# neptune-ai/open-solution-salt-identification

Hardware: AMD Instinct MI355X
Metric: training images/sec, U-Net ResNet34 101x101 (pad->128) bs32/GPU (higher is better)
Workload: dtype bf16; 1 GPU; architectures.unet.UNetResNet(34, hypercolumn) 128x128 (101 resized+edge-padded) batch 32/GPU, lovasz loss, Adam lr1e-4 L2 1e-4, train-mode BN; global_batch=32, parallelism=dp1

## Files before the change

### include/saltnet.h

```cpp
#ifndef SALTNET_H
#define SALTNET_H
#include <stdint.h>

#ifdef __cplusplus
extern "C" {
#endif

#define SALT_F32 0
#define SALT_BF16 1

#define SALT_OK 0
#define SALT_E_BADARG -1
#define SALT_E_UNSUPPORTED -2
#define SALT_E_LDS -3

#define SALT_MAX_TAPS 16

typedef struct {
    void* p;
    int B;
    int H;
    int W;
    int C;
    int cs;
// ... 14 lines not shown
    int in_step;
    int pad_mode;
    salt_view y;
    int OH;
    int OW;
    int out_step;
    int out_oy;
    int out_ox;
    const float* bias;
    const float* scale;
    const float* shift;
    int relu;
    int accumulate;
    float* stats;
    float* stats_cnt;
    int stats_part0;
    int cfg;
    void* strip;
    int strip_cs;
    int fold_top;
    int fold_bottom;
    int fold_left;
    int fold_right;
    salt_view bnb_y;
    salt_view bnb_a;
    const float* bnb_mean;
    const float* bnb_invstd;
    const float* bnb_gamma;
    const float* bnb_beta;
    float* bnb_partials;
    int bnb_relu;
    int nphase;
    int64_t w_phase_elems;
    const void* fin;
    double* fin_acc;
    uint32_t* fin_ticket;
    const void* bnb_fin;
    double* bnb_acc;
    uint32_t* bnb_ticket;
    salt_view res;
    const float* in_scale;
    const float* in_shift;
    int in_relu;
    const void* in_fin;
    const double* in_fin_acc;
    int64_t y_plane;
    int64_t x_plane;
} salt_conv_args;
int salt_conv(const salt_conv_args*, void* stream);
int salt_conv_stats_parts(const salt_conv_args*);
int salt_conv_kernel_id(const salt_conv_args*);
int salt_conv_tile_shape(const salt_conv_args*);

typedef struct {
    int dtype;
    salt_view p;
    salt_view q;
    int ntaps;
    int tap_dy[SALT_MAX_TAPS];
    int tap_dx[SALT_MAX_TAPS];
    int q_step;
    int pad_mode;
    float* partials;
    int nsplit;
    int64_t q_plane;
} salt_conv_wgrad_args;
// ... 715 lines not shown
```

### open-solution-salt-identification_amd/csrc/conv_mfma.hip

```cpp
#include <cstdlib>
#include <type_traits>
#include "common.h"
#ifndef SALT_K1_DBG
#define SALT_K1_DBG 0
#endif
#ifndef SALT_K1_FAST_STORE
#define SALT_K1_FAST_STORE 1
#endif

namespace {

struct ConvKP {
    const void* x; const void* w; void* y;
    const float* bias; const float* scale; const float* shift;
    float* stats; float* stats_cnt;
    int B, H, W, Cin, x_cs;
    int Cout, y_cs, OHf, OWf, OH, OW, out_step, out_oy, out_ox;
    int ntaps; int tap_off[SALT_MAX_TAPS];
    int in_step, pad_mode, min_dy, min_dx;
    int th_log2, tw_log2, nb;
    int gen, tw, th, twth;
    unsigned tw_magic, twth_magic;
    int hh, hw;
    int tiles_y, tiles_x;
    int nchunk, a_bytes;
    int relu, accumulate, stats_part0;
    void* strip; int strip_cs, fold_top, fold_bottom, fold_left, fold_right;
    int nphase, m_tiles_ph; int64_t w_phase_elems;
    int fold_fused, ox_shift;
    unsigned hhw_magic, hw_magic;
    int m_tiles, n_tiles;
    int vt;
    int nbuf;
    int no_perm8;
    int y_small;
    const void* bnb_y; const void* bnb_a; int bnb_cs, bnb_acs, bnb_relu;
    const float* bnb_mean; const float* bnb_invstd; const float* bnb_gamma; const float* bnb_beta; float* bnb_partials;
    const void* res; int res_cs;
    BnFin fin; BnbFin bnbf;
    const float* in_scale; const float* in_shift; int in_relu, in_tab_off; BnFin in_fin;
};

template <typename T> struct Mma;
template <> struct Mma<float> {
    static __device__ __forceinline__ void step(const u32x4& a, const u32x4& b, f32x16& c) {
        c = __builtin_amdgcn_mfma_f32_32x32x2f32(__uint_as_float(a.x), __uint_as_float(b.x), c, 0, 0, 0);
        c = __builtin_amdgcn_mfma_f32_32x32x2f32(__uint_as_float(a.y), __uint_as_float(b.y), c, 0, 0, 0);
        c = __builtin_amdgcn_mfma_f32_32x32x2f32(__uint_as_float(a.z), __uint_as_float(b.z), c, 0, 0, 0);
        c = __builtin_amdgcn_mfma_f32_32x32x2f32(__uint_as_float(a.w), __uint_as_float(b.w), c, 0, 0, 0);
    }
};
template <> struct Mma<bf16_t> {
    static __device__ __forceinline__ void step(const u32x4& a, const u32x4& b, f32x16& c) {
        c = __builtin_amdgcn_mfma_f32_32x32x16_bf16(__builtin_bit_cast(bf16x8, a), __builtin_bit_cast(bf16x8, b), c, 0, 0, 0);
    }
};

template <typename T>
__device__ __forceinline__ u32x4 load_piece(const T* base, int64_t off, int ch0, int C, bool vec_ok) {
    constexpr int VE = Elem<T>::VE;
    if (vec_ok && ch0 + VE <= C) return *reinterpret_cast<const u32x4*>(base + off);
    float f[VE];
#pragma unroll
    for (int j = 0; j < VE; ++j) f[j] = (ch0 + j < C) ? Elem<T>::ld(base + off + j) : 0.f;
    if (sizeof(T) == 4) return pack16<T>(f);
    return pack16<T>(f);
}

__device__ __forceinline__ int swz_addr(int row, int slot) {
    return row * 64 + (((slot ^ (row >> 2)) & 3) << 4);
}

struct TilePix { int tx, ty, bl; };
// ... 673 lines not shown
    switch (n) {
        case 0: asm volatile("s_waitcnt vmcnt(0)" ::: "memory"); break;
        case 1: asm volatile("s_waitcnt vmcnt(1)" ::: "memory"); break;
        case 2: asm volatile("s_waitcnt vmcnt(2)" ::: "memory"); break;
        case 3: asm volatile("s_waitcnt vmcnt(3)" ::: "memory"); break;
        case 4: asm volatile("s_waitcnt vmcnt(4)" ::: "memory"); break;
        case 5: asm volatile("s_waitcnt vmcnt(5)" ::: "memory"); break;
        case 6: asm volatile("s_waitcnt vmcnt(6)" ::: "memory"); break;
        case 7: asm volatile("s_waitcnt vmcnt(7)" ::: "memory"); break;
        case 8: asm volatile("s_waitcnt vmcnt(8)" ::: "memory"); break;
        case 9: asm volatile("s_waitcnt vmcnt(9)" ::: "memory"); break;
        case 10: asm volatile("s_waitcnt vmcnt(10)" ::: "memory"); break;
        case 11: asm volatile("s_waitcnt vmcnt(11)" ::: "memory"); break;
        case 12: asm volatile("s_waitcnt vmcnt(12)" ::: "memory"); break;
        case 13: asm volatile("s_waitcnt vmcnt(13)" ::: "memory"); break;
        case 14: asm volatile("s_waitcnt vmcnt(14)" ::: "memory"); break;
        case 15: asm volatile("s_waitcnt vmcnt(15)" ::: "memory"); break;
        case 16: asm volatile("s_waitcnt vmcnt(16)" ::: "memory"); break;
        case 17: asm volatile("s_waitcnt vmcnt(17)" ::: "memory"); break;
        case 18: asm volatile("s_waitcnt vmcnt(18)" ::: "memory"); break;
        default: asm volatile("s_waitcnt vmcnt(0)" ::: "memory"); break;
    }
}

typedef __attribute__((address_space(3))) void* lds_void_ptr;
typedef const __attribute__((address_space(1))) void* glb_void_ptr;

constexpr int v2_namax(int bm) { return bm <= 128 ? 13 : 25; }
#ifndef SALT_V2_DBG
#define SALT_V2_DBG 0
#endif
constexpr int DBG = SALT_V2_DBG;

template <int MI, int NI, int MB, int KS, int NT>
__global__ __launch_bounds__(512, 2) void conv_glds_kernel(ConvKP p) {
    constexpr int NAMAX = v2_namax(32 * MI * MB);
    typedef bf16_t T;
    static_assert(MB * KS == 8, "8 waves");
    static_assert(KS == 2 || KS == 4, "K slices");
    constexpr int NTHR = 512, VE = 8, KCE = 32;
    constexpr int BM = 32 * MI * MB, BN = 32 * NI;
    constexpr int NSUB = MI * NI;
    constexpr int OWN = NSUB >= KS ? NSUB / KS : 1;
    static_assert(NSUB >= KS ? (NSUB % KS == 0) : (KS % NSUB == 0), "slice reduction");
    constexpr int T0N = (NT + 1) / 2;
    extern __shared__ __attribute__((aligned(16))) unsigned char smem[];
    const int tid = threadIdx.x, lane = tid & 63;
    const int wave = __builtin_amdgcn_readfirstlane(tid >> 6);
    const int khalf = lane >> 5, l31 = lane & 31;
    const int mb = wave % MB, sl = wave / MB;
    const int taphalf = sl / (KS / 2), hsel = sl % (KS / 2);

    const int xcd = blockIdx.x & 7, local = blockIdx.x >> 3;
    const int n_tile = local % p.n_tiles;
    const int m_tile = (local / p.n_tiles) * 8 + xcd;
    if (m_tile >= p.m_tiles) return;
    int tile = m_tile, out_oy = p.out_oy, out_ox = p.out_ox;
    int64_t w_off = 0;
    if (p.nphase > 1) {
        const int ph = m_tile / p.m_tiles_ph;
        tile = m_tile - ph * p.m_tiles_ph;
        out_oy = ph >> 1; out_ox = ph & 1;
        w_off = ph * p.w_phase_elems;
    }
    const int txi = tile % p.tiles_x; tile /= p.tiles_x;
    const int tyi = tile % p.tiles_y;
    const int tbi = tile / p.tiles_y;
    const int oy0 = tyi * p.th, ox0 = txi * p.tw - p.ox_shift, b0 = tbi * p.nb;
    const int n0 = n_tile * BN;
    const int hhw = p.hh * p.hw;
    const int phalo = p.nb * hhw;
    const int iy0 = oy0 + p.min_dy, ix0 = ox0 + p.min_dx;
    const T* xg0 = reinterpret_cast<const T*>(p.x) + (int64_t)b0 * p.H * p.W * p.x_cs;
    const T* wg = reinterpret_cast<const T*>(p.w) + w_off;
    const unsigned char* zp = reinterpret_cast<const unsigned char*>(g_zero_piece);

    constexpr int NB_I = NT * BN / 16;
    constexpr int NS = (NAMAX + NB_I + 7) / 8;
    const int na = p.a_bytes >> 10;
    const int buf_bytes = p.a_bytes + NB_I * 1024;
    const int nbuf = p.nbuf;
    const int dummy_off = nbuf * buf_bytes + wave * 1024;
    const int w_chunk_bytes = NT * p.Cout * KCE * (int)sizeof(T);
    const unsigned char* d_src[NS];
    int d_inc[NS], d_off[NS];
#pragma unroll
    for (int i = 0; i < NS; ++i) {
        const int j = wave + 8 * i;
        d_src[i] = zp; d_inc[i] = 0; d_off[i] = -1;
        if (j < na) {
            d_off[i] = j * 1024;
            const int row = j * 16 + (lane >> 2);
            if (row < phalo) {
                const int bl = (int)__umulhi((unsigned)row, p.hhw_magic);
                const int r = row - bl * hhw;
                const int hy = (int)__umulhi((unsigned)r, p.hw_magic);
                const int hx = r - hy * p.hw;
                int iy = iy0 + hy, ix = ix0 + hx;
                bool valid = b0 + bl < p.B;
                if (p.pad_mode) { iy = min(max(iy, 0), p.H - 1); ix = min(max(ix, 0), p.W - 1); }
                else valid = valid && iy >= 0 && iy < p.H && ix >= 0 && ix < p.W;
                if (valid) {
                    const int slot = (lane ^ (row >> 2)) & 3;
                    d_src[i] = reinterpret_cast<const unsigned char*>(xg0 + ((bl * p.H + iy) * p.W + ix) * p.x_cs + slot * VE);
                    d_inc[i] = KCE * (int)sizeof(T);
                }
            }
        } else if (j < na + NB_I) {
            d_off[i] = p.a_bytes + (j - na) * 1024;
            const int row = (j - na) * 16 + (lane >> 2);
            const int t = row / BN, n = row - t * BN;
            if (n0 + n < p.Cout) {
                const int slot = (lane ^ (n >> 2)) & 3;
                d_src[i] = reinterpret_cast<const unsigned char*>(wg + ((int64_t)t * p.Cout + n0 + n) * KCE + slot * VE);
                d_inc[i] = w_chunk_bytes;
            }
        }
    }
    auto issue_slot = [&](int i, int buf, bool live) {
        if (DBG & 1) return;
        const bool real = live && d_off[i] >= 0;
        const int dst = real ? buf * buf_bytes + d_off[i] : dummy_off;
        const unsigned char* src = live ? d_src[i] : zp;
        __builtin_amdgcn_global_load_lds((glb_void_ptr)src, (lds_void_ptr)(smem + dst), 16, 0, 0);
        d_src[i] += d_inc[i];
    };

    const int perm = p.gen ? 0 : p.tw_log2 == 4 ? 1 : (MI % 2 == 0 && p.tw_log2 == 3 && p.th_log2 == 3 && p.hw == 10 && !p.no_perm8) ? 2 : 0;
    int pbase[MI];
#pragma unroll
    for (int i = 0; i < MI; ++i) {
        const int m = frag_pixel(perm, mb * MI + i, l31);
        const TilePix tp = tile_pix(p, m);
        const int tx = tp.tx, ty = tp.ty, bl = tp.bl;
        pbase[i] = bl < p.nb ? bl * hhw + ty * p.hw + tx : 0;
    }
    int b_addr[NI];
#pragma unroll
    for (int j = 0; j < NI; ++j) b_addr[j] = p.a_bytes + swz_addr(j * 32 + l31, khalf);

    f32x16 acc[MI][NI];
#pragma unroll
    for (int i = 0; i < MI; ++i)
#pragma unroll
        for (int j = 0; j < NI; ++j)
#pragma unroll
            for (int r = 0; r < 16; ++r) acc[i][j][r] = 0.f;

    struct Frag { u32x4 a[MI], b[NI]; };
    auto mma_frag = [&](const Frag& f) {
        if (DBG & 2) {
#pragma unroll
            for (int i = 0; i < MI; ++i)
#pragma unroll
                for (int j = 0; j < NI; ++j) acc[i][j][0] += __uint_as_float(f.a[i].x ^ f.b[j].y);
            return;
        }
#pragma unroll
        for (int i = 0; i < MI; ++i)
#pragma unroll
            for (int j = 0; j < NI; ++j)
                acc[i][j] = __builtin_amdgcn_mfma_f32_32x32x16_bf16(__builtin_bit_cast(bf16x8, f.a[i]), __builtin_bit_cast(bf16x8, f.b[j]), acc[i][j], 0, 0, 0);
    };

    auto run = [&](auto ta_c, auto tb_c) {
        constexpr int TA = decltype(ta_c)::value, TB = decltype(tb_c)::value, NTL = TB - TA;
        constexpr int NST = NTL * (KS == 2 ? 2 : 1);
        int a_addr[NTL][MI];
// ... 32 lines not shown
            asm volatile("" ::: "memory");
            __builtin_amdgcn_s_barrier();
            asm volatile("" ::: "memory");
            const bool live = c + nbuf - 1 < p.nchunk;
            const int fill = slot_i;
            slot_i = (slot_i + 1 == nbuf) ? 0 : slot_i + 1;
            const unsigned char* base = smem + slot_c * buf_bytes;
            slot_c = (slot_c + 1 == nbuf) ? 0 : slot_c + 1;
            Frag f0, f1;
            load_frag(0, base, f0);
            __builtin_amdgcn_sched_group_barrier(0x100, MI + NI, 0);
            constexpr int SPS = (NS + NST - 1) / NST;
#pragma unroll
            for (int s = 0; s < NST; s += 2) {
                if (s + 1 < NST) load_frag(s + 1, base, f1);
#pragma unroll
                for (int u = 0; u < SPS; ++u) if (s * SPS + u < NS) issue_slot(s * SPS + u, fill, live);
                mma_frag(f0);
                if (s + 1 < NST) __builtin_amdgcn_sched_group_barrier(0x100, MI + NI, 0);
                if (!(DBG & 1)) __builtin_amdgcn_sched_group_barrier(0x010, SPS, 0);
                __builtin_amdgcn_sched_group_barrier(0x008, MI * NI, 0);
                if (s + 1 < NST) {
                    if (s + 2 < NST) load_frag(s + 2, base, f0);
#pragma unroll
                    for (int u = 0; u < SPS; ++u) if ((s + 1) * SPS + u < NS) issue_slot((s + 1) * SPS + u, fill, live);
                    mma_frag(f1);
                    if (s + 2 < NST) __builtin_amdgcn_sched_group_barrier(0x100, MI + NI, 0);
                    if (!(DBG & 1)) __builtin_amdgcn_sched_group_barrier(0x010, SPS, 0);
                    __builtin_amdgcn_sched_group_barrier(0x008, MI * NI, 0);
                }
            }
        }
    };
    if (DBG & 16) { if (tid == 0 && blockIdx.x == 0x7fffffff) reinterpret_cast<int*>(p.y)[0] = pbase[0] + (int)(size_t)d_src[0] + d_off[1] + b_addr[0]; return; }
    if (taphalf == 0) run(std::integral_constant<int, 0>{}, std::integral_constant<int, T0N>{});
    else run(std::integral_constant<int, T0N>{}, std::integral_constant<int, NT>{});
    if (DBG & 8) {
        float tsum = 0.f;
#pragma unroll
        for (int i = 0; i < MI; ++i)
#pragma unroll
            for (int j = 0; j < NI; ++j)
#pragma unroll
                for (int r = 0; r < 16; ++r) tsum += acc[i][j][r];
        if (tsum == 123.456f) reinterpret_cast<float*>(p.y)[0] = tsum;
        return;
    }

    f32x16 fin[OWN];
    int rowoff[OWN], coloff[OWN];
    bool owner;
    {
        float* red = reinterpret_cast<float*>(smem);
        asm volatile("s_waitcnt vmcnt(0)" ::: "memory");
        __syncthreads();
#pragma unroll
        for (int i = 0; i < MI; ++i)
#pragma unroll
            for (int j = 0; j < NI; ++j) {
                const int u = i * NI + j;
                const int own_sl = NSUB >= KS ? (u % KS) : u;
                if (sl != own_sl) {
                    float* dst = red + ((((mb * NSUB + u) * KS + sl) * 16) * 64) + lane * 4;
#pragma unroll
                    for (int r4 = 0; r4 < 4; ++r4) {
                        const f32x4 v = {acc[i][j][r4 * 4], acc[i][j][r4 * 4 + 1], acc[i][j][r4 * 4 + 2], acc[i][j][r4 * 4 + 3]};
                        *reinterpret_cast<f32x4*>(dst + r4 * 256) = v;
                    }
// ... 301 lines not shown
        salt_view yv = a->y, xv = a->x;
        if (a->y_plane) yv.cs = yv.C;
        if (a->x_plane) xv.cs = xv.C;
        if (!view_ok(xv) || !view_ok(yv) || !a->w) SALT_FAIL(SALT_E_BADARG, "conv: bad view");
        if (a->y_plane < 0 || a->x_plane < 0) SALT_FAIL(SALT_E_BADARG, "conv: x_plane / y_plane");
    }
    if (a->ntaps < 1 || a->ntaps > SALT_MAX_TAPS) SALT_FAIL(SALT_E_BADARG, "conv: ntaps %d", a->ntaps);
    if (a->in_step < 1 || a->in_step > 2 || a->out_step < 1 || a->out_step > 2) SALT_FAIL(SALT_E_BADARG, "conv: steps");
    if (a->OH < 1 || a->OW < 1) SALT_FAIL(SALT_E_BADARG, "conv: empty output grid");
    const bool fold_fused = !a->strip && (a->fold_top > 0 || a->fold_right > 0);
    if (fold_fused) {
        const int ve = a->dtype == SALT_F32 ? 4 : 8;
        if (a->fold_bottom || a->fold_left || a->fold_top < 0 || a->fold_right < 0 || a->out_step != 1 || a->out_oy || a->out_ox || a->stats || a->fin_acc ||
            a->OH != a->y.H + a->fold_top || a->OW != a->y.W + a->fold_right)
            SALT_FAIL(SALT_E_BADARG, "conv: fused fold needs OH/OW = y.H + top / y.W + right (top / right pads only), out_step 1, no stats");
        if (a->y.C % ve || a->y.cs % ve || (reinterpret_cast<uintptr_t>(a->y.p) & 15))
            SALT_FAIL(SALT_E_BADARG, "conv: fused fold needs 16-byte aligned whole channel pieces");
    }
    if (!a->strip && !fold_fused && ((a->OH - 1) * a->out_step + a->out_oy >= a->y.H || (a->OW - 1) * a->out_step + a->out_ox >= a->y.W))
        SALT_FAIL(SALT_E_BADARG, "conv: output grid exceeds buffer");
    if (a->x.B != a->y.B) SALT_FAIL(SALT_E_BADARG, "conv: batch mismatch");
    const int Cout = a->y.C;
    int min_dy = 1 << 30, max_dy = -(1 << 30), min_dx = 1 << 30, max_dx = -(1 << 30);
    for (int t = 0; t < a->ntaps; ++t) {
        min_dy = a->tap_dy[t] < min_dy ? a->tap_dy[t] : min_dy; max_dy = a->tap_dy[t] > max_dy ? a->tap_dy[t] : max_dy;
        min_dx = a->tap_dx[t] < min_dx ? a->tap_dx[t] : min_dx; max_dx = a->tap_dx[t] > max_dx ? a->tap_dx[t] : max_dx;
    }
    const int64_t pixels = (int64_t)a->x.B * a->OH * a->OW * (a->nphase > 1 ? a->nphase : 1);
    const int KCE_ = a->dtype == SALT_F32 ? 16 : 32;
    static const bool vt_off = getenv("SALT_CONV_NO_VT") != nullptr;
    const int vt = (!vt_off && a->ntaps == 1 && a->in_step == 1 && a->x.C % (4 * KCE_) == 0) ? 4 : 1;
    static const int v2_env = getenv("SALT_CONV_V2") ? atoi(getenv("SALT_CONV_V2")) : 1;
    const bool in_tf = a->in_scale || a->in_fin_acc;
    const bool v2_ok = a->dtype == SALT_BF16 && a->in_step == 1 && (a->ntaps == 9 || a->ntaps == 4) && a->x.C % 32 == 0 &&
                       a->x.cs % 8 == 0 && (reinterpret_cast<uintptr_t>(a->x.p) & 15) == 0 && !in_tf;
    int id = ((a->cfg & 0xff) >= 9 && (a->cfg & 0xff) <= 13) ? 0 : (a->cfg & 0xff);
    if (id >= 6 && !v2_ok) id = 0;
    if (id == 2 && vt > 1) id = 1;
    if (id == 0 && v2_ok && v2_env && ((a->cfg & 0xff) == 0 || ((a->cfg & 0xff) >= 9 && (a->cfg & 0xff) <= 13))) {
        if (v2_env >= 6) id = v2_env;
        else {
            const int64_t t256 = ((pixels + 255) / 256) * cdiv(Cout, 64), t128 = ((pixels + 127) / 128) * cdiv(Cout, 64);
            if (t128 < 192 && Cout > 32) id = 8;
            else if (v2_env >= 2 && t256 < 256 && Cout > 32) id = 7;
            else if (v2_env >= 3) id = Cout <= 32 ? 8 : (t256 >= 256 ? 6 : 7);
        }
    }
    if (id == 0) {
        const bool big = a->in_step == 1 && a->OH >= 16 && a->OW >= 16 && pixels >= 256 * 256 * 2;
        if (Cout <= 32) id = 4;
        else if (big && vt == 1) id = 2;
        else id = 1;
        const int64_t wgs = ((pixels + 127) / 128) * cdiv(Cout, 64);
        static const int small_cfg = getenv("SALT_CONV_SMALL_CFG") ? atoi(getenv("SALT_CONV_SMALL_CFG")) : 4;
        if (id == 1 && wgs < 512) id = (small_cfg == 5 && wgs >= 256) ? 1 : small_cfg;
    }
    const TileCfg* cfg = nullptr;
    for (const auto& c : kCfgs) if (c.id == id) cfg = &c;
    if (!cfg) SALT_FAIL(SALT_E_BADARG, "conv: unknown cfg %d", id);
    for (int attempt = 0; attempt < 4; ++attempt) {
        const int BM = 32 * cfg->MI * cfg->WM;
        ConvKP& k = pl->kp;
        k.tw_log2 = ilog2_ceil(a->OW) < 4 ? ilog2_ceil(a->OW) : 4;
        int rem = ilog2_ceil(BM) - k.tw_log2;
        k.th_log2 = ilog2_ceil(a->OH) < rem ? ilog2_ceil(a->OH) : rem;
        k.nb = BM >> (k.tw_log2 + k.th_log2);
        int th = 1 << k.th_log2, tw = 1 << k.tw_log2;
        k.gen = 0;
        static const bool gen_off = getenv("SALT_CONV_GEN_TILES") && atoi(getenv("SALT_CONV_GEN_TILES")) == 0;
        if (fold_fused && !gen_off && a->in_step == 1 && vt == 1 && a->OW * (a->fold_top + 1) <= BM) {
            const int gtw = a->OW;
            int gth = BM / gtw, gnb = 1;
            if (gth >= a->OH) { gth = a->OH; gnb = BM / (a->OH * a->OW); }
            const int64_t slots_p2 = (int64_t)cdiv(a->x.B, k.nb) * cdiv(a->OH, th) * cdiv(a->OW, tw) * BM;
            const int64_t slots_g = (int64_t)cdiv(a->x.B, gnb) * cdiv(a->OH, gth) * BM;
            const int gphalo = gnb * (gth + max_dy - min_dy) * (gtw + max_dx - min_dx);
            const bool fits = cfg->KS > 0 ? cdiv(gphalo, 16) <= v2_namax(BM) : gphalo * 4 <= maxa_for(BM) * 256;
            if (fits && slots_g * 115 <= slots_p2 * 100) {
                k.gen = 1; th = gth; tw = gtw; k.nb = gnb; k.tw_log2 = 0; k.th_log2 = 0;
            }
        }
        k.tw = tw; k.th = th; k.twth = tw * th;
        k.tw_magic = (unsigned)((1ull << 32) / (unsigned)tw) + 1u; k.twth_magic = (unsigned)((1ull << 32) / (unsigned)(tw * th)) + 1u;
        k.hh = (th - 1) * a->in_step + (max_dy - min_dy) + 1;
        k.hw = (tw - 1) * a->in_step + (max_dx - min_dx) + 1;
        const int phalo = k.nb * k.hh * k.hw * vt;
        if (cfg->KS > 0) {
            const int64_t buf = (int64_t)cdiv(phalo, 16) * 1024 + (int64_t)a->ntaps * (32 * cfg->NI) * 64;
            k.nbuf = 3 * buf + 8192 <= 160 * 1024 ? 3 : 2;
            static const bool no_perm8 = getenv("SALT_GLDS_NO_PERM8") != nullptr;
            k.no_perm8 = no_perm8 ? 1 : 0;
            if (cdiv(phalo, 16) > v2_namax(BM) || 2 * buf + 8192 > 160 * 1024) {
                if (attempt == 0 && cfg->id != 8) { for (const auto& c : kCfgs) if (c.id == 8) cfg = &c; continue; }
                if ((a->cfg & 0xff) < 6) { for (const auto& c : kCfgs) if (c.id == 4) cfg = &c; continue; }
                SALT_FAIL(SALT_E_UNSUPPORTED, "conv: halo tile of %d pixels too large for the LDS ring", phalo);
            }
            break;
        }
        if (phalo * 4 > maxa_for(BM) * 256) {
            if (cfg->id != 5) { for (const auto& c : kCfgs) if (c.id == 5) cfg = &c; continue; }
            SALT_FAIL(SALT_E_UNSUPPORTED, "conv: halo tile of %d pixels too large", phalo);
        }
        break;
    }
    pl->cfg = *cfg;
    ConvKP& k = pl->kp;
    const int BN = 32 * cfg->NI * cfg->WN;
    const int KCE = a->dtype == SALT_F32 ? 16 : 32;
    k.x = a->x.p; k.w = a->w; k.y = a->y.p;
    k.bias = a->bias; k.scale = a->scale; k.shift = a->shift; k.stats = a->stats; k.stats_cnt = a->stats_cnt;
    k.B = a->x.B; k.H = a->x.H; k.W = a->x.W; k.Cin = a->x.C; k.x_cs = a->x.cs;
    k.Cout = Cout; k.y_cs = a->y.cs; k.OHf = a->y.H; k.OWf = a->y.W; k.OH = a->OH; k.OW = a->OW;
    k.out_step = a->out_step; k.out_oy = a->out_oy; k.out_ox = a->out_ox;
    k.ntaps = a->ntaps; k.in_step = a->in_step; k.pad_mode = a->pad_mode; k.min_dy = min_dy; k.min_dx = min_dx;
    for (int t = 0; t < a->ntaps; ++t) k.tap_off[t] = (a->tap_dy[t] - min_dy) * k.hw + (a->tap_dx[t] - min_dx);
    k.vt = vt;
    if (vt > 1) { k.ntaps = vt; for (int t = 0; t < vt; ++t) k.tap_off[t] = t * k.nb * k.hh * k.hw; }
    k.fold_fused = fold_fused ? 1 : 0;
    k.tiles_y = cdiv(a->OH, k.th); k.tiles_x = cdiv(a->OW, k.tw);
    k.ox_shift = (fold_fused && a->fold_right > 0) ? k.tiles_x * k.tw - a->OW : 0;
    if (fold_fused && (k.th <= a->fold_top || k.tw <= a->fold_right))
        SALT_FAIL(SALT_E_UNSUPPORTED, "conv: fused fold needs tiles larger than the pad (%d x %d)", k.th, k.tw);
    const int tiles_b = cdiv(a->x.B, k.nb);
    k.nchunk = cdiv(a->x.C, KCE * vt);
    k.a_bytes = k.nb * k.hh * k.hw * 64 * vt;
    if (cfg->KS > 0) k.a_bytes = cdiv(k.nb * k.hh * k.hw, 16) * 1024;
    k.hhw_magic = (unsigned)((1ull << 32) / (unsigned)(k.hh * k.hw)) + 1u;
    k.hw_magic = (unsigned)((1ull << 32) / (unsigned)k.hw) + 1u;
    k.relu = a->relu; k.accumulate = a->accumulate; k.stats_part0 = a->stats_part0;
    k.strip = a->strip; k.strip_cs = a->strip_cs; k.fold_top = a->fold_top; k.fold_bottom = a->fold_bottom; k.fold_left = a->fold_left; k.fold_right = a->fold_right;
    k.m_tiles = tiles_b * k.tiles_y * k.tiles_x; k.n_tiles = cdiv(Cout, BN);
    k.nphase = a->nphase > 1 ? a->nphase : 1; k.m_tiles_ph = k.m_tiles; k.w_phase_elems = a->w_phase_elems;
    if (k.nphase > 1) {
        if (k.nphase != 4 || a->out_step != 2 || a->strip || fold_fused || a->w_phase_elems <= 0 ||
            (a->OH - 1) * 2 + 1 >= a->y.H || (a->OW - 1) * 2 + 1 >= a->y.W)
            SALT_FAIL(SALT_E_BADARG, "conv: a phase-fused launch is 4 output-parity phases of an out_step 2 grid that fits y for every parity");
        k.m_tiles *= 4;
    }
    pl->grid = dim3((unsigned)(cdiv(k.m_tiles, 8) * 8 * k.n_tiles), 1, 1);
    pl->lds = (size_t)k.a_bytes + (size_t)k.ntaps * BN * 64;
    if (cfg->KS > 0) {
        pl->lds = pl->lds * (size_t)k.nbuf + 8192;
        const size_t red = (size_t)cfg->WM * (cfg->MI * cfg->NI) * cfg->KS * 4096;
        if (red > pl->lds) pl->lds = red;
    }
    {
        const size_t es = a->dtype == SALT_F32 ? 4 : 2;
        size_t out_bytes = (size_t)(32 * cfg->MI * cfg->WM) * (BN * es + 16);
        if (cfg->KS == 0 && (a->stats || a->fin_acc)) out_bytes += 16 + (size_t)cfg->WM * BN * 8 + (size_t)cfg->WM * 4 + 32;
        if (out_bytes > pl->lds) pl->lds = out_bytes;
    }
    pl->parts = tiles_b * k.tiles_y * k.tiles_x * k.nphase;
    k.bnb_partials = a->bnb_partials; k.bnb_y = a->bnb_y.p; k.bnb_cs = a->bnb_y.cs; k.bnb_relu = a->bnb_relu;
    k.bnb_a = a->bnb_a.p; k.bnb_acs = a->bnb_a.cs;
    k.bnb_mean = a->bnb_mean; k.bnb_invstd = a->bnb_invstd; k.bnb_gamma = a->bnb_gamma; k.bnb_beta = a->bnb_beta;
    if (a->bnb_partials || a->bnb_acc) {
        const int ve = a->dtype == SALT_F32 ? 4 : 8;
        const bool all_phases = k.nphase == 4 && a->out_step == 2 && !a->out_oy && !a->out_ox && a->OH * 2 == a->y.H && a->OW * 2 == a->y.W;
        if (a->strip || a->stats || a->fin_acc || ((a->out_step != 1 || a->out_oy || a->out_ox) && !all_phases) ||
            (!fold_fused && !all_phases && (a->OH != a->y.H || a->OW != a->y.W)))
            SALT_FAIL(SALT_E_BADARG, "conv: BatchNorm-backward sums need a plain (or fused-fold, or all-phases stride-2) full-grid launch");
        if (!view_ok(a->bnb_y) || a->bnb_y.B != a->y.B || a->bnb_y.H != a->y.H || a->bnb_y.W != a->y.W || a->bnb_y.C != a->y.C)
            SALT_FAIL(SALT_E_BADARG, "conv: bnb_y shape");
        if (!a->bnb_mean || !a->bnb_invstd || !a->bnb_gamma || !a->bnb_beta) SALT_FAIL(SALT_E_BADARG, "conv: bnb parameters missing");
        if (a->bnb_a.p && (!view_ok(a->bnb_a) || a->bnb_a.B != a->y.B || a->bnb_a.H != a->y.H || a->bnb_a.W != a->y.W || a->bnb_a.C != a->y.C ||
// ... 88 lines not shown
            else {
                if (npa <= 3) return launch_cfg_nt<T, MI, NI, WM, WN, 9, 3, true>(pl, st);
                return launch_cfg_nt<T, MI, NI, WM, WN, 9, 9, true>(pl, st);
            }
            SALT_FAIL(SALT_E_UNSUPPORTED, "conv: the input transform does not fit this tile's loader");
        }
        if (ok && k.ntaps == 9) {
            if constexpr (MI * WM == 8) { if (npa <= 6) return launch_cfg_nt<T, MI, NI, WM, WN, 9, 6>(pl, st); }
            else {
                if (npa <= 3) return launch_cfg_nt<T, MI, NI, WM, WN, 9, 3>(pl, st);
                return launch_cfg_nt<T, MI, NI, WM, WN, 9, 9>(pl, st);
            }
        }
        if constexpr (MI * WM != 8) { if (ok && k.ntaps == 4) return launch_cfg_nt<T, MI, NI, WM, WN, 4, 9>(pl, st); }
    }
    if (pl.kp.in_scale || pl.kp.in_fin.acc) SALT_FAIL(SALT_E_UNSUPPORTED, "conv: the input transform needs bf16 tiles of 128 or 256 pixels");
    if (pl.kp.ntaps == 9) return launch_cfg_nt<T, MI, NI, WM, WN, 9>(pl, st);
    if (pl.kp.ntaps == 4) return launch_cfg_nt<T, MI, NI, WM, WN, 4>(pl, st);
    return launch_cfg_nt<T, MI, NI, WM, WN, 0>(pl, st);
}

template <int MI, int NI, int MB, int KS>
int launch_glds(const Plan& pl, hipStream_t st) {
    auto go = [&](auto kern, bool& attr_set) -> int {
        if (!attr_set) {
            hipError_t e = hipFuncSetAttribute(reinterpret_cast<const void*>(kern), hipFuncAttributeMaxDynamicSharedMemorySize, 160 * 1024);
            if (e != hipSuccess) SALT_FAIL((int)e, "hipFuncSetAttribute: %s", hipGetErrorString(e));
            attr_set = true;
        }
        hipLaunchKernelGGL(kern, pl.grid, dim3(512), pl.lds, st, pl.kp);
        SALT_CHECK_LAUNCH();
        return SALT_OK;
    };
    static bool set9 = false, set4 = false;
    if (pl.kp.ntaps == 9) return go(conv_glds_kernel<MI, NI, MB, KS, 9>, set9);
    return go(conv_glds_kernel<MI, NI, MB, KS, 4>, set4);
}

template <typename T>
int launch_T(const Plan& pl, hipStream_t st) {
    if constexpr (sizeof(T) == 2) {
        switch (pl.cfg.id) {
            case 6: return launch_glds<2, 2, 4, 2>(pl, st);
            case 7: return launch_glds<2, 2, 2, 4>(pl, st);
            case 8: return launch_glds<2, 1, 2, 4>(pl, st);
        }
    }
    switch (pl.cfg.id) {
        case 1: return launch_cfg<T, 2, 1, 2, 2>(pl, st);
        case 2: return launch_cfg<T, 2, 2, 4, 1>(pl, st);
        case 3: return launch_cfg<T, 2, 2, 2, 2>(pl, st);
        case 4: return launch_cfg<T, 1, 1, 4, 1>(pl, st);
        case 5: return launch_cfg<T, 1, 1, 2, 2>(pl, st);
    }
    SALT_FAIL(SALT_E_BADARG, "conv: cfg");
}

struct PackKP {
    const float* w; void* wp; int D0, D1, KH, KW, ntaps, transpose, N, C, nchunk;
    int n_off, n_total, chunk_off;
    int tap_kh[SALT_MAX_TAPS], tap_kw[SALT_MAX_TAPS];
};
template <typename T>
__global__ void pack_weight_kernel(PackKP p) {
    constexpr int KCE = 64 / (int)sizeof(T);
    const int64_t total = (int64_t)p.nchunk * p.ntaps * p.N * KCE;
    T* out = reinterpret_cast<T*>(p.wp);
// ... 1517 lines not shown
```

### open-solution-salt-identification_amd/csrc/runtime.hip

```cpp
#include <stdarg.h>
#include <string.h>
#include <stdlib.h>
#include "common.h"

static thread_local char g_err[512] = "";

void salt_set_error(const char* fmt, ...) {
    va_list ap;
    va_start(ap, fmt);
    vsnprintf(g_err, sizeof(g_err), fmt, ap);
    va_end(ap);
}

extern "C" const char* salt_last_error(void) { return g_err; }

extern "C" int salt_abi_version(void) { return 25; }

extern "C" int salt_device_info(int* cu_count, int* lds_bytes, char* arch_name, int arch_name_len) {
    int dev = 0;
    hipError_t e = hipGetDevice(&dev);
    if (e != hipSuccess) SALT_FAIL((int)e, "hipGetDevice: %s", hipGetErrorString(e));
    hipDeviceProp_t prop;
    e = hipGetDeviceProperties(&prop, dev);
    if (e != hipSuccess) SALT_FAIL((int)e, "hipGetDeviceProperties: %s", hipGetErrorString(e));
    if (cu_count) *cu_count = prop.multiProcessorCount;
    if (lds_bytes) *lds_bytes = (int)prop.sharedMemPerBlock;
    if (arch_name && arch_name_len > 0) { strncpy(arch_name, prop.gcnArchName, arch_name_len - 1); arch_name[arch_name_len - 1] = 0; }
    return SALT_OK;
}

extern "C" int salt_program_run_range(const salt_program_entry* e, int begin, int end, void* stream) {
    if (!e || begin < 0 || end < begin) SALT_FAIL(SALT_E_BADARG, "program: bad range");
    for (int i = begin; i < end; ++i) {
        const int rc = e[i].fn(e[i].args, stream);
        if (rc) {
            char prev[400];
            strncpy(prev, g_err, sizeof(prev) - 1); prev[sizeof(prev) - 1] = 0;
            salt_set_error("program entry %d failed (%d): %s", i, rc, prev);
            return rc;
        }
    }
    return SALT_OK;
}

extern "C" int salt_program_run_timed(const salt_program_entry* e, int begin, int end, void* stream, float* ms_out) {
    if (!e || begin < 0 || end < begin || !ms_out) SALT_FAIL(SALT_E_BADARG, "program: bad range");
    const int n = end - begin;
    hipStream_t st = (hipStream_t)stream;
    hipEvent_t* ev = new hipEvent_t[n + 1];
// ... 328 lines not shown
```

### open-solution-salt-identification_amd/engine.py

```python
import ctypes
import os

import numpy as np
import torch

from ._abi import OP_FUNCS, STRUCTS, SaltError, check, fill, lib

DT_CODE = {'f32': 0, 'bf16': 1}
TORCH_DT = {'f32': torch.float32, 'bf16': torch.bfloat16}
VEC = {'f32': 4, 'bf16': 8}


def fwd_bn_fold():
    return os.environ.get('SALT_FWD_BN_FOLD', '0') not in ('', '0')


def _round_up(v, m):
    return (v + m - 1) // m * m


class Scratch:

    def __init__(self, name, nbytes):
        self.name, self.nbytes = name, int(nbytes)
# ... 945 lines not shown
                nbytes = x.B * Hp * Wp * ext.cs * self._es()
                self._conv_launch(self.bwd, dy.gview(), pk.data_ptr(), td, 1, 0, (ext, Scratch('dgrad_ext', nbytes)), Hp, Wp, stream=self._bwd_pack_tag())
                self.bwd.add('pad_fold', dtype=self.dt, xp=(ext, Scratch('dgrad_ext', nbytes)), top=top, bottom=0, left=0, right=right,
                             x=x.gview(), accumulate=acc)
                return
            if x.C % self.ve == 0 and not os.environ.get('SALT_FOLD_STRIP'):
                s = self._conv_launch(self.bwd, dy.gview(), pk.data_ptr(), td, 1, 0, x.gview(), Hp, Wp, accumulate=acc,
                                      fold_top=top, fold_right=right, stream=self._bwd_pack_tag())
                if not x.plane_stride():
                    x.buf.grad_writers[-1][2] = s
                return
            scs = _round_up(x.C, self.ve)
            ring = lib.salt_fold_strip_pixels(x.H, x.W, top, 0, 0, right)
            strip = Scratch('dgrad_ring', x.B * ring * scs * self._es())
            self._conv_launch(self.bwd, dy.gview(), pk.data_ptr(), td, 1, 0, x.gview(), Hp, Wp, accumulate=acc,
                              strip=strip, strip_cs=scs, fold_top=top, fold_right=right, stream=self._bwd_pack_tag())
            self.bwd.add('pad_fold_strip', dtype=self.dt, strip=strip, strip_cs=scs, top=top, bottom=0, left=0, right=right, x=x.gview())
            return
        acc = x.grad_state()
        if stride == 1:
            td = [(-t[2], -t[3]) for t in taps]
            s = self._conv_launch(self.bwd, dy.gview(), pk.data_ptr(), td, 1, 0, x.gview(), x.H, x.W, accumulate=acc, stream=self._bwd_pack_tag())
            if not x.plane_stride():
                x.buf.grad_writers[-1][2] = s
            return
        phases = []
        for ay in range(2):
            for ax in range(2):
                sel = [i for i, t in enumerate(taps) if (t[2] - ay) % 2 == 0 and (t[3] - ax) % 2 == 0]
                phases.append((ay, ax, sel))
        fused = self._phase_fused([[(((ay - taps[i][2]) // 2, (ax - taps[i][3]) // 2), tk[i]) for i in sel] for ay, ax, sel in phases], x.H, x.W)
        if fused is not None:
            td_u, phase_taps = fused
            pk_t, elems = eng.packed_phases(conv, phase_taps, transposed=True, bwd=True)
            s = self._conv_launch(self.bwd, dy.gview(), pk_t.data_ptr(), td_u, 1, 0, x.gview(), x.H // 2, x.W // 2, out_step=2, accumulate=acc,
                                  nphase=4, w_phase_elems=elems, stream=self._bwd_pack_tag())
            if not x.plane_stride() and not os.environ.get('SALT_NO_BNB_PHASE'):
                x.buf.grad_writers[-1][2] = s
            return
        if any(not sel for _, _, sel in phases) and not acc:
            self.fill(x, 0.0, grad=True)
            acc = 1
        for ay, ax, sel in phases:
            oh, ow = (x.H - ay + 1) // 2, (x.W - ax + 1) // 2
            if not sel or oh <= 0 or ow <= 0:
                continue
            pk_s = eng.packed(conv, [tk[i] for i in sel], transposed=True, bwd=True)
            td = [((ay - taps[i][2]) // 2, (ax - taps[i][3]) // 2) for i in sel]
            self._conv_launch(self.bwd, dy.gview(), pk_s.data_ptr(), td, 1, 0, x.gview(), oh, ow, out_step=2, out_oy=ay, out_ox=ax, accumulate=acc,
                              stream=self._bwd_pack_tag())

    def _phase_fused(self, per_phase, H, W):
        if os.environ.get('SALT_NO_PHASE_FUSE') or H % 2 or W % 2:
            return None
        offs = sorted({o for ph in per_phase for o, _ in ph})
        if not offs or len(offs) > 9 or sum(1 for ph in per_phase if ph) < 2:
            return None
        if 4 * len(offs) > 1.8 * sum(len(ph) for ph in per_phase):
            return None
        if len(offs) not in (4, 9):
            offs = offs + [offs[0]] * ((4 if len(offs) < 4 else 9) - len(offs))
        phase_taps = []
        for ph in per_phase:
            d = dict(ph)
            used = set()
            row = []
            for o in offs:
                if o in d and o not in used:
                    row.append(d[o]); used.add(o)
# ... 386 lines not shown
```

Before: 6353 images/s.

## Add stride-2 GLDS conv path and skip dead taps in phase-fused backward

Adds a STEP=2 variant of the LDS-ring MFMA conv kernel. It gathers stride-2 inputs through a deinterleaved halo layout (even columns first, then odd), so 3x3 stride-2 convs can use the fast v2 path instead of the fallback kernel. For phase-fused transposed backward convs, tap order is rearranged and a per-phase live-tap mask is passed in. Waves whose tap half holds only zero weights then skip the MFMA work and only keep the load/barrier cadence. In exchange, the stride-2 variant has a larger halo budget and a launch bound of 1, which reduces occupancy, and it adds more template instantiations.

```diff
diff --git a/include/saltnet.h b/include/saltnet.h
--- a/include/saltnet.h
+++ b/include/saltnet.h
@@ -70,6 +70,7 @@
     int bnb_relu;
     int nphase;
     int64_t w_phase_elems;
+    int phase_live;
     const void* fin;
     double* fin_acc;
     uint32_t* fin_ticket;
diff --git a/open-solution-salt-identification_amd/csrc/conv_mfma.hip b/open-solution-salt-identification_amd/csrc/conv_mfma.hip
--- a/open-solution-salt-identification_amd/csrc/conv_mfma.hip
+++ b/open-solution-salt-identification_amd/csrc/conv_mfma.hip
@@ -39,6 +39,8 @@
     const void* res; int res_cs;
     BnFin fin; BnbFin bnbf;
     const float* in_scale; const float* in_shift; int in_relu, in_tab_off; BnFin in_fin;
+    int deint_ne;
+    int phase_live;
 };
 
 template <typename T> struct Mma;
@@ -778,9 +780,11 @@
 #endif
 constexpr int DBG = SALT_V2_DBG;
 
-template <int MI, int NI, int MB, int KS, int NT>
-__global__ __launch_bounds__(512, 2) void conv_glds_kernel(ConvKP p) {
-    constexpr int NAMAX = v2_namax(32 * MI * MB);
+constexpr int glds_namax(int bm, int step) { return step == 2 && bm <= 128 ? 37 : v2_namax(bm); }
+
+template <int MI, int NI, int MB, int KS, int NT, int STEP = 1>
+__global__ __launch_bounds__(512, STEP == 2 ? 1 : 2) void conv_glds_kernel(ConvKP p) {
+    constexpr int NAMAX = glds_namax(32 * MI * MB, STEP);
     typedef bf16_t T;
     static_assert(MB * KS == 8, "8 waves");
     static_assert(KS == 2 || KS == 4, "K slices");
@@ -803,11 +807,14 @@
     if (m_tile >= p.m_tiles) return;
     int tile = m_tile, out_oy = p.out_oy, out_ox = p.out_ox;
     int64_t w_off = 0;
+    int live = (1 << NT) - 1;
     if (p.nphase > 1) {
-        const int ph = m_tile / p.m_tiles_ph;
-        tile = m_tile - ph * p.m_tiles_ph;
+        const int pq = m_tile / p.m_tiles_ph;
+        tile = m_tile - pq * p.m_tiles_ph;
+        const int ph = p.phase_live ? 3 - pq : pq;
         out_oy = ph >> 1; out_ox = ph & 1;
         w_off = ph * p.w_phase_elems;
+        if (p.phase_live) live = (p.phase_live >> (4 * ph)) & 0xf;
     }
     const int txi = tile % p.tiles_x; tile /= p.tiles_x;
     const int tyi = tile % p.tiles_y;
@@ -816,7 +823,7 @@
     const int n0 = n_tile * BN;
     const int hhw = p.hh * p.hw;
     const int phalo = p.nb * hhw;
-    const int iy0 = oy0 + p.min_dy, ix0 = ox0 + p.min_dx;
+    const int iy0 = oy0 * STEP + p.min_dy, ix0 = ox0 * STEP + p.min_dx;
     const T* xg0 = reinterpret_cast<const T*>(p.x) + (int64_t)b0 * p.H * p.W * p.x_cs;
     const T* wg = reinterpret_cast<const T*>(p.w) + w_off;
     const unsigned char* zp = reinterpret_cast<const unsigned char*>(g_zero_piece);
@@ -841,7 +848,8 @@
                 const int bl = (int)__umulhi((unsigned)row, p.hhw_magic);
                 const int r = row - bl * hhw;
                 const int hy = (int)__umulhi((unsigned)r, p.hw_magic);
-                const int hx = r - hy * p.hw;
+                int hx = r - hy * p.hw;
+                if (STEP == 2) hx = hx < p.deint_ne ? 2 * hx : 2 * (hx - p.deint_ne) + 1;
                 int iy = iy0 + hy, ix = ix0 + hx;
                 bool valid = b0 + bl < p.B;
                 if (p.pad_mode) { iy = min(max(iy, 0), p.H - 1); ix = min(max(ix, 0), p.W - 1); }
@@ -856,7 +864,7 @@
             d_off[i] = p.a_bytes + (j - na) * 1024;
             const int row = (j - na) * 16 + (lane >> 2);
             const int t = row / BN, n = row - t * BN;
-            if (n0 + n < p.Cout) {
+            if (n0 + n < p.Cout && ((live >> t) & 1)) {
                 const int slot = (lane ^ (n >> 2)) & 3;
                 d_src[i] = reinterpret_cast<const unsigned char*>(wg + ((int64_t)t * p.Cout + n0 + n) * KCE + slot * VE);
                 d_inc[i] = w_chunk_bytes;
@@ -872,14 +880,15 @@
         d_src[i] += d_inc[i];
     };
 
-    const int perm = p.gen ? 0 : p.tw_log2 == 4 ? 1 : (MI % 2 == 0 && p.tw_log2 == 3 && p.th_log2 == 3 && p.hw == 10 && !p.no_perm8) ? 2 : 0;
+    const int perm = p.gen ? 0 : p.tw_log2 == 4 ? 1 :
+                     (MI % 2 == 0 && p.tw_log2 == 3 && p.th_log2 == 3 && STEP * p.hw == (STEP == 2 ? 34 : 10) && !p.no_perm8) ? 2 : 0;
     int pbase[MI];
 #pragma unroll
     for (int i = 0; i < MI; ++i) {
         const int m = frag_pixel(perm, mb * MI + i, l31);
         const TilePix tp = tile_pix(p, m);
         const int tx = tp.tx, ty = tp.ty, bl = tp.bl;
-        pbase[i] = bl < p.nb ? bl * hhw + ty * p.hw + tx : 0;
+        pbase[i] = bl < p.nb ? bl * hhw + ty * STEP * p.hw + tx : 0;
     }
     int b_addr[NI];
 #pragma unroll
@@ -978,8 +987,40 @@
             }
         }
     };
+    auto idle = [&]() {
+#pragma unroll 1
+        for (int c0 = 0; c0 < nbuf - 1; ++c0) {
+            const bool lv = c0 < p.nchunk;
+#pragma unroll
+            for (int i = 0; i < NS; ++i) issue_slot(i, c0, lv);
+        }
+        int slot_i = nbuf - 1;
+        for (int c = 0; c < p.nchunk; ++c) {
+            if (!(DBG & 1)) {
+                if (nbuf == 3) asm volatile("s_waitcnt vmcnt(%0)" :: "n"(NS) : "memory");
+                else asm volatile("s_waitcnt vmcnt(0)" ::: "memory");
+            }
+            asm volatile("" ::: "memory");
+            __builtin_amdgcn_s_barrier();
+            asm volatile("" ::: "memory");
+            const bool lv = c + nbuf - 1 < p.nchunk;
+#pragma unroll
+            for (int i = 0; i < NS; ++i) issue_slot(i, slot_i, lv);
+            slot_i = (slot_i + 1 == nbuf) ? 0 : slot_i + 1;
+        }
+    };
     if (DBG & 16) { if (tid == 0 && blockIdx.x == 0x7fffffff) reinterpret_cast<int*>(p.y)[0] = pbase[0] + (int)(size_t)d_src[0] + d_off[1] + b_addr[0]; return; }
-    if (taphalf == 0) run(std::integral_constant<int, 0>{}, std::integral_constant<int, T0N>{});
+    using I0 = std::integral_constant<int, 0>;
+    using I1 = std::integral_constant<int, 1>;
+    using I2 = std::integral_constant<int, 2>;
+    using I3 = std::integral_constant<int, 3>;
+    using I4 = std::integral_constant<int, 4>;
+    if (NT == 4 && live != 0xf) {
+        const int hm = (live >> (2 * taphalf)) & 3;
+        if (hm == 0) idle();
+        else if (taphalf == 0) { if (hm == 3) run(I0{}, I2{}); else if (hm == 1) run(I0{}, I1{}); else run(I1{}, I2{}); }
+        else { if (hm == 3) run(I2{}, I4{}); else if (hm == 1) run(I2{}, I3{}); else run(I3{}, I4{}); }
+    } else if (taphalf == 0) run(std::integral_constant<int, 0>{}, std::integral_constant<int, T0N>{});
     else run(std::integral_constant<int, T0N>{}, std::integral_constant<int, NT>{});
     if (DBG & 8) {
         float tsum = 0.f;
@@ -1347,14 +1388,19 @@
     const int vt = (!vt_off && a->ntaps == 1 && a->in_step == 1 && a->x.C % (4 * KCE_) == 0) ? 4 : 1;
     static const int v2_env = getenv("SALT_CONV_V2") ? atoi(getenv("SALT_CONV_V2")) : 1;
     const bool in_tf = a->in_scale || a->in_fin_acc;
-    const bool v2_ok = a->dtype == SALT_BF16 && a->in_step == 1 && (a->ntaps == 9 || a->ntaps == 4) && a->x.C % 32 == 0 &&
+    static const bool s2_on = !(getenv("SALT_CONV_S2") && atoi(getenv("SALT_CONV_S2")) == 0);
+    const bool s2 = a->in_step == 2 && a->ntaps == 9 && s2_on;
+    const bool v2_ok = a->dtype == SALT_BF16 && (a->in_step == 1 ? (a->ntaps == 9 || a->ntaps == 4) : s2) && a->x.C % 32 == 0 &&
                        a->x.cs % 8 == 0 && (reinterpret_cast<uintptr_t>(a->x.p) & 15) == 0 && !in_tf;
+    const bool live_ph = s2_on && a->phase_live && a->nphase == 4 && a->ntaps == 4 && a->x.C >= 16 * 32;
     int id = ((a->cfg & 0xff) >= 9 && (a->cfg & 0xff) <= 13) ? 0 : (a->cfg & 0xff);
     if (id >= 6 && !v2_ok) id = 0;
+    if (id >= 6 && a->in_step == 2) id = 7;
     if (id == 2 && vt > 1) id = 1;
     if (id == 0 && v2_ok && v2_env && ((a->cfg & 0xff) == 0 || ((a->cfg & 0xff) >= 9 && (a->cfg & 0xff) <= 13))) {
-        if (v2_env >= 6) id = v2_env;
-        else {
+        if (v2_env >= 6) id = s2 ? 7 : v2_env;
+        else if (live_ph) id = 8;
+        else if (!s2) {
             const int64_t t256 = ((pixels + 255) / 256) * cdiv(Cout, 64), t128 = ((pixels + 127) / 128) * cdiv(Cout, 64);
             if (t128 < 192 && Cout > 32) id = 8;
             else if (v2_env >= 2 && t256 < 256 && Cout > 32) id = 7;
@@ -1405,8 +1451,9 @@
             k.nbuf = 3 * buf + 8192 <= 160 * 1024 ? 3 : 2;
             static const bool no_perm8 = getenv("SALT_GLDS_NO_PERM8") != nullptr;
             k.no_perm8 = no_perm8 ? 1 : 0;
-            if (cdiv(phalo, 16) > v2_namax(BM) || 2 * buf + 8192 > 160 * 1024) {
-                if (attempt == 0 && cfg->id != 8) { for (const auto& c : kCfgs) if (c.id == 8) cfg = &c; continue; }
+            if (cdiv(phalo, 16) > glds_namax(BM, a->in_step) || 2 * buf + 8192 > 160 * 1024) {
+                const int alt = a->in_step == 2 ? 7 : 8;
+                if (attempt == 0 && cfg->id != alt) { for (const auto& c : kCfgs) if (c.id == alt) cfg = &c; continue; }
                 if ((a->cfg & 0xff) < 6) { for (const auto& c : kCfgs) if (c.id == 4) cfg = &c; continue; }
                 SALT_FAIL(SALT_E_UNSUPPORTED, "conv: halo tile of %d pixels too large for the LDS ring", phalo);
             }
@@ -1429,6 +1476,14 @@
     k.out_step = a->out_step; k.out_oy = a->out_oy; k.out_ox = a->out_ox;
     k.ntaps = a->ntaps; k.in_step = a->in_step; k.pad_mode = a->pad_mode; k.min_dy = min_dy; k.min_dx = min_dx;
     for (int t = 0; t < a->ntaps; ++t) k.tap_off[t] = (a->tap_dy[t] - min_dy) * k.hw + (a->tap_dx[t] - min_dx);
+    k.deint_ne = 0;
+    if (cfg->KS > 0 && a->in_step == 2) {
+        k.deint_ne = (k.hw + 1) / 2;
+        for (int t = 0; t < a->ntaps; ++t) {
+            const int u = a->tap_dx[t] - min_dx;
+            k.tap_off[t] = (a->tap_dy[t] - min_dy) * k.hw + ((u & 1) ? k.deint_ne + (u >> 1) : (u >> 1));
+        }
+    }
     k.vt = vt;
     if (vt > 1) { k.ntaps = vt; for (int t = 0; t < vt; ++t) k.tap_off[t] = t * k.nb * k.hh * k.hw; }
     k.fold_fused = fold_fused ? 1 : 0;
@@ -1446,6 +1501,7 @@
     k.strip = a->strip; k.strip_cs = a->strip_cs; k.fold_top = a->fold_top; k.fold_bottom = a->fold_bottom; k.fold_left = a->fold_left; k.fold_right = a->fold_right;
     k.m_tiles = tiles_b * k.tiles_y * k.tiles_x; k.n_tiles = cdiv(Cout, BN);
     k.nphase = a->nphase > 1 ? a->nphase : 1; k.m_tiles_ph = k.m_tiles; k.w_phase_elems = a->w_phase_elems;
+    k.phase_live = (live_ph && cfg->KS > 0 && (a->phase_live & 0xffff) != 0xffff) ? (a->phase_live & 0xffff) : 0;
     if (k.nphase > 1) {
         if (k.nphase != 4 || a->out_step != 2 || a->strip || fold_fused || a->w_phase_elems <= 0 ||
             (a->OH - 1) * 2 + 1 >= a->y.H || (a->OW - 1) * 2 + 1 >= a->y.W)
@@ -1600,7 +1656,11 @@
         SALT_CHECK_LAUNCH();
         return SALT_OK;
     };
-    static bool set9 = false, set4 = false;
+    static bool set9 = false, set4 = false, set9s2 = false;
+    if constexpr (32 * MI * MB == 128 && NI == 2) {
+        if (pl.kp.in_step == 2) return go(conv_glds_kernel<MI, NI, MB, KS, 9, 2>, set9s2);
+    }
+    if (pl.kp.in_step != 1) SALT_FAIL(SALT_E_BADARG, "conv_glds: stride %d", pl.kp.in_step);
     if (pl.kp.ntaps == 9) return go(conv_glds_kernel<MI, NI, MB, KS, 9>, set9);
     return go(conv_glds_kernel<MI, NI, MB, KS, 4>, set4);
 }
diff --git a/open-solution-salt-identification_amd/csrc/runtime.hip b/open-solution-salt-identification_amd/csrc/runtime.hip
--- a/open-solution-salt-identification_amd/csrc/runtime.hip
+++ b/open-solution-salt-identification_amd/csrc/runtime.hip
@@ -14,7 +14,7 @@
 
 extern "C" const char* salt_last_error(void) { return g_err; }
 
-extern "C" int salt_abi_version(void) { return 25; }
+extern "C" int salt_abi_version(void) { return 26; }
 
 extern "C" int salt_device_info(int* cu_count, int* lds_bytes, char* arch_name, int arch_name_len) {
     int dev = 0;
diff --git a/open-solution-salt-identification_amd/engine.py b/open-solution-salt-identification_amd/engine.py
--- a/open-solution-salt-identification_amd/engine.py
+++ b/open-solution-salt-identification_amd/engine.py
@@ -1001,9 +1001,15 @@
         fused = self._phase_fused([[(((ay - taps[i][2]) // 2, (ax - taps[i][3]) // 2), tk[i]) for i in sel] for ay, ax, sel in phases], x.H, x.W)
         if fused is not None:
             td_u, phase_taps = fused
+            live = 0
+            if self.dtype == 'bf16' and os.environ.get('SALT_CONV_S2') != '0' and sorted(td_u) == [(0, 0), (0, 1), (1, 0), (1, 1)]:
+                order = [td_u.index(o) for o in [(0, 0), (1, 1), (0, 1), (1, 0)]]
+                td_u = [td_u[i] for i in order]
+                phase_taps = [[row[i] for i in order] for row in phase_taps]
+                live = sum(1 << (4 * ph + t) for ph, row in enumerate(phase_taps) for t, kk in enumerate(row) if kk is not None)
             pk_t, elems = eng.packed_phases(conv, phase_taps, transposed=True, bwd=True)
             s = self._conv_launch(self.bwd, dy.gview(), pk_t.data_ptr(), td_u, 1, 0, x.gview(), x.H // 2, x.W // 2, out_step=2, accumulate=acc,
-                                  nphase=4, w_phase_elems=elems, stream=self._bwd_pack_tag())
+                                  nphase=4, w_phase_elems=elems, phase_live=live, stream=self._bwd_pack_tag())
             if not x.plane_stride() and not os.environ.get('SALT_NO_BNB_PHASE'):
                 x.buf.grad_writers[-1][2] = s
             return
```

Result: no change. 6323 images/s, median of 2 (-0.5%).
